# meyerls/FruitNeRF

Measured on AMD Instinct MI355X. Metric: train rays/sec, fruit_nerf on synthetic apple 800x800, higher is better.
Workload: dtype f32 fwd (MLP GEMMs: 3-piece bf16 split, 6 products, ~2^-24) / 2-piece bwd (dX, dW: 3 products, ~2^-17; its forward recompute 3-piece); everything else f32

## Files before the change

### fruitnerf_amd/csrc/field_bf16.hpp

```cpp
#pragma once
#include "field_layers.hpp"

namespace fnr {

using bf16x8 = __attribute__((ext_vector_type(8))) __bf16;
using f32x8 = __attribute__((ext_vector_type(8))) float;

enum { MLP_FP32 = 0, MLP_BF16 = 1, MLP_BF16X3 = 3 };

template <class Cfg>
struct BfImage {
  static constexpr int NL = Cfg::NLAYERS;
  static constexpr int nib_used(int l) { return l == Cfg::L_COL0 ? Cfg::HB : Cfg::nib(l); }
  static constexpr int nkb(int l) { return (nib_used(l) + 1) / 2; }
  static constexpr int nkbT(int l) { return (Cfg::nob(l) + 1) / 2; }
  static constexpr bool hasT(int l) { return l != Cfg::L_SEM0; }
  static constexpr int fblocks(int l) { return Cfg::nob(l) * nkb(l); }
  static constexpr int tblocks(int l) { return hasT(l) ? nib_used(l) * nkbT(l) : 0; }
  static constexpr int foff(int l) {
    int o = 0;
    for (int i = 0; i < l; ++i) o += fblocks(i);
    return o;
  }
  static constexpr int F_TOTAL = foff(NL);
  static constexpr int toff(int l) {
    int o = F_TOTAL;
    for (int i = 0; i < l; ++i) o += tblocks(i);
    return o;
  }
  static constexpr int BLOCKS = toff(NL);
  static constexpr size_t piece_elems() { return (size_t)BLOCKS * 64 * 8; }
  static constexpr size_t bytes(int ns) { return (size_t)ns * piece_elems() * 2; }
};
constexpr int BF_MAX_PIECES = 3;

__device__ __forceinline__ __bf16 bf_piece(float w, int p) {
  const __bf16 a = (__bf16)w;
  if (p == 0) return a;
  const float r1 = w - (float)a;
  const __bf16 b = (__bf16)r1;
  if (p == 1) return b;
  return (__bf16)(r1 - (float)b);
}

template <class Cfg>
__device__ __forceinline__ void pack_field_weights_bf16_block(const FieldPtrs& p, int ns, __bf16* __restrict__ image,
                                                              int block) {
  using Img = BfImage<Cfg>;
  const int idx = block * 256 + threadIdx.x;
  if (idx >= Img::BLOCKS * 64) return;
  const int blk = idx >> 6, lane = idx & 63;
  const int i = lane & 15, g = lane >> 4;
  float w[8];
  if (blk < Img::F_TOTAL) {
    int l = 0;
#pragma unroll
    for (int q = 1; q < Cfg::NLAYERS; ++q)
      if (blk >= Img::foff(q)) l = q;
    const int local = blk - Img::foff(l);
    const int nkb = Img::nkb(l), kb = local % nkb, ob = local / nkb;
    const int out = 16 * ob + i;
#pragma unroll
    for (int e = 0; e < 8; ++e) {
      const int ib = 2 * kb + (e >> 2);
      const int col = (ib < Img::nib_used(l)) ? kmap<Cfg>(Cfg::km(l), ib, g, e & 3, Cfg::in_dim(l)) : -1;
      w[e] = (out < Cfg::out_dim(l) && col >= 0) ? p.w[l][out * Cfg::in_dim(l) + col] : 0.0f;
    }
  } else {
    int l = 0;
#pragma unroll
    for (int q = 1; q < Cfg::NLAYERS; ++q)
      if (blk >= Img::toff(q)) l = q;
    const int local = blk - Img::toff(l);
    const int nk = Img::nkbT(l), kb = local % nk, ib = local / nk;
    const int col = kmap<Cfg>(Cfg::km(l), ib, i >> 2, i & 3, Cfg::in_dim(l));
#pragma unroll
    for (int e = 0; e < 8; ++e) {
      const int ob = 2 * kb + (e >> 2);
      const int out = 16 * ob + 4 * g + (e & 3);
      w[e] = (ob < Cfg::nob(l) && out < Cfg::out_dim(l) && col >= 0) ? p.w[l][out * Cfg::in_dim(l) + col] : 0.0f;
    }
  }
  for (int pc = 0; pc < ns; ++pc) {
    bf16x8 v;
#pragma unroll
    for (int e = 0; e < 8; ++e) v[e] = bf_piece(w[e], pc);
    reinterpret_cast<bf16x8*>(image)[(size_t)pc * Img::BLOCKS * 64 + idx] = v;
  }
}

template <class Cfg>
__global__ __launch_bounds__(256) void k_pack_field_weights_bf16(FieldPtrs p, int ns, __bf16* __restrict__ image) {
  pack_field_weights_bf16_block<Cfg>(p, ns, image, blockIdx.x);
}
template <class Cfg>
constexpr int pack_field_weights_bf16_blocks() { return (BfImage<Cfg>::BLOCKS * 64 + 255) / 256; }

template <class Cfg>
static inline void launch_pack_field_weights_bf16(const FieldPtrs& p, int ns, __bf16* image, hipStream_t st) {
  hipLaunchKernelGGL((k_pack_field_weights_bf16<Cfg>), dim3(pack_field_weights_bf16_blocks<Cfg>()), dim3(256), 0, st, p, ns,
                     image);
}

template <class Cfg>
__global__ __launch_bounds__(256) void k_prepare_field(FieldPtrs p, float* __restrict__ packed, int ns,
                                                       __bf16* __restrict__ image, RaysDev rays,
                                                       const float* __restrict__ embedding,
                                                       const float* __restrict__ mean_embedding,
                                                       float* __restrict__ ray_bias, int nb_pack, int nb_pack16) {
  int b = blockIdx.x;
  if (b < nb_pack) {
    pack_field_weights_block<Cfg>(p, packed, b);
    return;
  }
  b -= nb_pack;
  if (b < nb_pack16) {
    pack_field_weights_bf16_block<Cfg>(p, ns, image, b);
    return;
  }
  b -= nb_pack16;
  color_ray_bias_block<Cfg, true>(p, nullptr, rays, embedding, mean_embedding, ray_bias, b,
                                  (int)gridDim.x - nb_pack - nb_pack16);
}
template <class Cfg>
static inline void launch_prepare_field(const FieldPtrs& p, float* packed, int ns, __bf16* image, const RaysDev& rays,
                                        const float* embedding, const float* mean_embedding, float* ray_bias,
                                        hipStream_t st) {
  const int nb_pack = pack_field_weights_blocks<Cfg>();
  const int nb_pack16 = ns > 0 ? pack_field_weights_bf16_blocks<Cfg>() : 0;
  const long long nb_bias = color_ray_bias_blocks(rays);
  hipLaunchKernelGGL((k_prepare_field<Cfg>), dim3((unsigned)(nb_pack + nb_pack16 + nb_bias)), dim3(256), 0, st, p, packed, ns,
                     image, rays, embedding, mean_embedding, ray_bias, nb_pack, nb_pack16);
}

template <class Cfg, class Segs, int NS>
struct BfLds {
  using Img = BfImage<Cfg>;
  static constexpr int blocks(int s) { return Segs::isT(s) ? Img::tblocks(Segs::layer(s)) : Img::fblocks(Segs::layer(s)); }
  static constexpr int off(int s) {
    int o = 0;
    for (int i = 0; i < s; ++i) o += blocks(i) * NS;
    return o;
  }
  static constexpr int FRAGS = off(Segs::N);
  static constexpr int BYTES = FRAGS * 1024;
  static constexpr int find(int layer, bool isT) {
    for (int i = 0; i < Segs::N; ++i)
      if (Segs::layer(i) == layer && Segs::isT(i) == isT) return i;
    return -1;
  }
  template <int LAYER, bool IS_T>
  __device__ static __forceinline__ const bf16x8* seg(const bf16x8* lds) {
    constexpr int s = find(LAYER, IS_T);
    static_assert(s >= 0, "layer not staged by this kernel");
    return lds + off(s) * 64;
  }
  template <int LAYER, bool IS_T>
  static constexpr int seg_blocks() { return blocks(find(LAYER, IS_T)); }
  static constexpr int chunk_begin(int c) { return off(c / NS) * 64 + (c % NS) * blocks(c / NS) * 64; }
  static constexpr long long chunk_src(int c) {
    const int s = c / NS, pc = c % NS;
    return (long long)pc * Img::BLOCKS * 64 + (Segs::isT(s) ? Img::toff(Segs::layer(s)) : Img::foff(Segs::layer(s))) * 64;
  }
  template <int THREADS>
  __device__ static __forceinline__ void stage(bf16x8* __restrict__ lds, const __bf16* __restrict__ image) {
    constexpr int T = FRAGS * 64, NCH = Segs::N * NS;
    constexpr int PER = (T + THREADS - 1) / THREADS;
    static_assert(PER <= 32, "staging batch too large");
    const f32x4* img = reinterpret_cast<const f32x4*>(image);
    f32x4* dst = reinterpret_cast<f32x4*>(lds);
    f32x4 v[PER];
#pragma unroll
    for (int u = 0; u < PER; ++u) {
      const int f = (int)threadIdx.x + u * THREADS;
      long long delta = chunk_src(0) - chunk_begin(0);
#pragma unroll
      for (int c = 1; c < NCH; ++c) delta = (f >= chunk_begin(c)) ? chunk_src(c) - chunk_begin(c) : delta;
      if (f < T) v[u] = img[f + delta];
    }
#pragma unroll
    for (int u = 0; u < PER; ++u) {
      const int f = (int)threadIdx.x + u * THREADS;
      if (f < T) dst[f] = v[u];
    }
  }
};

template <class Cfg, int L, int NS, int THREADS>
__device__ __forceinline__ void bf_build_T(bf16x8* __restrict__ lds, const float* __restrict__ packed) {
  constexpr int NIB = Cfg::nib(L), NKT = (Cfg::nob(L) + 1) / 2, TB = NIB * NKT;
  for (int idx = threadIdx.x; idx < TB * 64; idx += THREADS) {
    const int blk = idx >> 6, lane = idx & 63;
    const int i = lane & 15, g = lane >> 4;
    const int kb = blk % NKT, ib = blk / NKT;
    float w[8];
#pragma unroll
    for (int e = 0; e < 8; ++e) {
      const int ob = 2 * kb + (e >> 2), row = 4 * g + (e & 3);
      w[e] = ob < Cfg::nob(L) ? packed[Cfg::woff(L) + ((ob * NIB + ib) * 64 + swz_slot(row, i >> 2)) * 4 + (i & 3)] : 0.0f;
    }
#pragma unroll
    for (int pc = 0; pc < NS; ++pc) {
      bf16x8 v;
#pragma unroll
      for (int e = 0; e < 8; ++e) v[e] = bf_piece(w[e], pc);
      lds[pc * TB * 64 + idx] = v;
    }
  }
}

using bf_f32x2 = __attribute__((ext_vector_type(2))) float;
using bf_bf16x2 = __attribute__((ext_vector_type(2))) __bf16;
__device__ __forceinline__ unsigned cvt_pk_bf16(float lo, float hi) {
  const bf_f32x2 v = {lo, hi};
  return __builtin_bit_cast(unsigned, __builtin_convertvector(v, bf_bf16x2));
}
using bf_u32x4 = __attribute__((ext_vector_type(4))) unsigned;
template <int NS>
__device__ __forceinline__ void bf_split(const f32x8 v, bf16x8 (&p)[NS]) {
  bf_u32x4 out[NS];
#pragma unroll
  for (int d = 0; d < 4; ++d) {
    float a = v[2 * d], b = v[2 * d + 1];
#pragma unroll
    for (int pc = 0; pc < NS; ++pc) {
      const unsigned w = cvt_pk_bf16(a, b);
      out[pc][d] = w;
      if (pc + 1 < NS) {
        a -= __builtin_bit_cast(float, w << 16);
        b -= __builtin_bit_cast(float, w & 0xffff0000u);
      }
    }
  }
#pragma unroll
  for (int pc = 0; pc < NS; ++pc) p[pc] = __builtin_bit_cast(bf16x8, out[pc]);
}
template <int NS>
__device__ __forceinline__ void bf_split_half(const f32x4 v, bf16x8 (&p)[NS]) {
  bf_u32x4 out[NS];
#pragma unroll
  for (int d = 0; d < 2; ++d) {
    float a = v[2 * d], b = v[2 * d + 1];
#pragma unroll
    for (int pc = 0; pc < NS; ++pc) {
      const unsigned w = cvt_pk_bf16(a, b);
      out[pc][d] = w;
      if (pc + 1 < NS) {
        a -= __builtin_bit_cast(float, w << 16);
        b -= __builtin_bit_cast(float, w & 0xffff0000u);
      }
    }
  }
#pragma unroll
  for (int pc = 0; pc < NS; ++pc) {
    out[pc][2] = out[pc][3] = 0u;
    p[pc] = __builtin_bit_cast(bf16x8, out[pc]);
  }
}

template <int NS, int NB>
__device__ __forceinline__ void bf_operand(const f32x4 (&act)[NB], bf16x8 (&x)[(NB + 1) / 2][NS]) {
#pragma unroll
  for (int kb = 0; kb < (NB + 1) / 2; ++kb) {
    if (2 * kb + 1 < NB) {
      f32x8 v;
#pragma unroll
      for (int e = 0; e < 4; ++e) {
        v[e] = act[2 * kb][e];
        v[4 + e] = act[(2 * kb + 1 < NB) ? 2 * kb + 1 : 0][e];
      }
      bf_split<NS>(v, x[kb]);
    } else {
      bf_split_half<NS>(act[2 * kb], x[kb]);
    }
  }
}

template <int NS, int NOB, int NKB>
__device__ __forceinline__ void bf_layer_acc(const bf16x8* __restrict__ seg, const bf16x8 (&xa)[NKB][NS],
                                             const bf16x8 (&xb)[NKB][NS], f32x4 (&oa)[NOB], f32x4 (&ob_)[NOB], int lane) {
  constexpr int PB = NOB * NKB * 64;
#pragma unroll
  for (int kb = 0; kb < NKB; ++kb) {
#pragma unroll
    for (int ob = 0; ob < NOB; ++ob) {
      bf16x8 w[NS];
#pragma unroll
      for (int pc = 0; pc < NS; ++pc) w[pc] = seg[pc * PB + (ob * NKB + kb) * 64 + lane];
#pragma unroll
      for (int s = NS - 1; s >= 0; --s)
#pragma unroll
        for (int pw = 0; pw <= s; ++pw) {
          oa[ob] = __builtin_amdgcn_mfma_f32_16x16x32_bf16(w[pw], xa[kb][s - pw], oa[ob], 0, 0, 0);
          ob_[ob] = __builtin_amdgcn_mfma_f32_16x16x32_bf16(w[pw], xb[kb][s - pw], ob_[ob], 0, 0, 0);
        }
    }
  }
}

template <int NS, int NOB, int NIB>
__device__ __forceinline__ void bf_layer(const bf16x8* __restrict__ seg, const float* __restrict__ B,
                                         const f32x4 (&ina)[NIB], const f32x4 (&inb)[NIB], f32x4 (&oa)[NOB],
                                         f32x4 (&ob_)[NOB], int lane) {
  const int g = lane >> 4;
#pragma unroll
  for (int ob = 0; ob < NOB; ++ob) oa[ob] = ob_[ob] = *reinterpret_cast<const f32x4*>(B + 16 * ob + 4 * g);
  bf16x8 xa[(NIB + 1) / 2][NS], xb[(NIB + 1) / 2][NS];
  bf_operand<NS, NIB>(ina, xa);
  bf_operand<NS, NIB>(inb, xb);
  bf_layer_acc<NS, NOB, (NIB + 1) / 2>(seg, xa, xb, oa, ob_, lane);
}

template <int NS, int NIBO, int NOB>
__device__ __forceinline__ void bf_layer_T(const bf16x8* __restrict__ segT, const f32x4 (&Ga)[NOB], const f32x4 (&Gb)[NOB],
                                           f32x4 (&oa)[NIBO], f32x4 (&ob_)[NIBO], int lane) {
#pragma unroll
  for (int ib = 0; ib < NIBO; ++ib) oa[ib] = ob_[ib] = f32x4{0.f, 0.f, 0.f, 0.f};
  bf16x8 xa[(NOB + 1) / 2][NS], xb[(NOB + 1) / 2][NS];
  bf_operand<NS, NOB>(Ga, xa);
  bf_operand<NS, NOB>(Gb, xb);
  bf_layer_acc<NS, NIBO, (NOB + 1) / 2>(segT, xa, xb, oa, ob_, lane);
}

template <int NS, int NOB, int NKB>
__device__ __forceinline__ void bf_layer_acc1(const bf16x8* __restrict__ seg, const bf16x8 (&x)[NKB][NS], f32x4 (&o)[NOB],
                                              int lane) {
  constexpr int PB = NOB * NKB * 64, T = NOB * NKB;
  bf16x8 w[2][NS];
  auto load = [&](int t, bf16x8 (&dst)[NS]) {
    const int kb = t / NOB, ob = t % NOB;
#pragma unroll
    for (int pc = 0; pc < NS; ++pc) dst[pc] = seg[pc * PB + (ob * NKB + kb) * 64 + lane];
  };
  load(0, w[0]);
#pragma unroll
  for (int t = 0; t < T; ++t) {
    if (t + 1 < T) load(t + 1, w[(t + 1) & 1]);
    const int kb = t / NOB, ob = t % NOB;
#pragma unroll
    for (int s = NS - 1; s >= 0; --s)
#pragma unroll
      for (int pw = 0; pw <= s; ++pw)
        o[ob] = __builtin_amdgcn_mfma_f32_16x16x32_bf16(w[t & 1][pw], x[kb][s - pw], o[ob], 0, 0, 0);
    __builtin_amdgcn_sched_barrier(0);
  }
}
template <int NS, int NOB, int NIB>
__device__ __forceinline__ void bf_layer1(const bf16x8* __restrict__ seg, const float* __restrict__ B,
                                          const f32x4 (&in)[NIB], f32x4 (&o)[NOB], int lane) {
  const int g = lane >> 4;
#pragma unroll
  for (int ob = 0; ob < NOB; ++ob) o[ob] = *reinterpret_cast<const f32x4*>(B + 16 * ob + 4 * g);
  bf16x8 x[(NIB + 1) / 2][NS];
  bf_operand<NS, NIB>(in, x);
  bf_layer_acc1<NS, NOB, (NIB + 1) / 2>(seg, x, o, lane);
}
template <int NS, int NIBO, int NOB>
__device__ __forceinline__ void bf_layer_T1(const bf16x8* __restrict__ segT, const f32x4 (&G)[NOB], f32x4 (&o)[NIBO],
                                            int lane) {
#pragma unroll
  for (int ib = 0; ib < NIBO; ++ib) o[ib] = f32x4{0.f, 0.f, 0.f, 0.f};
  bf16x8 x[(NOB + 1) / 2][NS];
  bf_operand<NS, NOB>(G, x);
  bf_layer_acc1<NS, NIBO, (NOB + 1) / 2>(segT, x, o, lane);
}

size_t field_bf16_image_bytes();
int field_mlp_fwd_bf16(int cfg, int mode, const FieldPtrs& p, const float* packed, void* image_ws, const float* ray_bias,
                       const RaysDev& rd, int S, long long N, const float2* feats, const uint8_t* selector, float* density,
                       float* rgb, float* logit, float* geo_out, float* h_buf, hipStream_t st);
int field_mlp_fwd_sem_big_bf16(int mode, const FieldPtrs& p, void* image_ws, const float* packed, long long N,
                               const float* h_buf, float* logit, hipStream_t st);
int field_mlp_bwd_sem_big_bf16(int mode, const FieldPtrs& p, void* image_ws, const float* packed, long long N,
                               const float* h_saved, const float* d_logit, float* partials, long long blocks,
                               hipStream_t st, float* d_h_semgrad = nullptr);
namespace pw {
struct BwdArgs {
  const float* packed;
  const __bf16* image;
  const float* ray_bias;
  RaysDev rd;
  int S;
  long long N;
  const float2* feats;
  const float* h_saved;
  const uint8_t* selector;
  const float *d_density, *d_rgb, *d_logit;
  float2* d_feats;
  float *d_h, *gsum_tile, *gsum_extra, *partials;
  long long blocks;
  hipStream_t st;
};
}
int field_mlp_bwd_pw(int cfg, int mode, int branch, const pw::BwdArgs& a, const float2* jac, float4* d_pos);

}
```

### fruitnerf_amd/csrc/field_mlp_bf16.hip

```cpp
#include <type_traits>

#include "field_bf16.hpp"

namespace fnr {

template <class Cfg>
struct SegsFwdAll {
  static constexpr int N = Cfg::NLAYERS;
  static constexpr int layer(int i) { return i; }
  static constexpr bool isT(int) { return false; }
};

template <class Cfg>
struct SegsFwdBaseColor {
  static constexpr int N = 5;
  static constexpr int layer(int i) {
    return i == 0 ? Cfg::L_BASE0 : i == 1 ? Cfg::L_BASE1 : i == 2 ? Cfg::L_COL0 : i == 3 ? Cfg::L_COL1 : Cfg::L_COL2;
  }
  static constexpr bool isT(int) { return false; }
};

__device__ __forceinline__ void load_hash_block(const float2* __restrict__ feats, long long N, long long nn, int g,
                                                f32x4 (&x0)[2]) {
#pragma unroll
  for (int m = 0; m < 4; ++m) {
    const float2 v = feats[(size_t)(4 * m + g) * N + nn];
    x0[m >> 1][2 * (m & 1)] = v.x;
    x0[m >> 1][2 * (m & 1) + 1] = v.y;
  }
}

template <int N>
__device__ __forceinline__ void relu2_(f32x4 (&a)[N], f32x4 (&b)[N]) {
  relu_(a);
  relu_(b);
}

template <class Cfg, int NS, int WAVES, bool WITH_SEM>
__global__ __launch_bounds__(64 * WAVES, WAVES / 4) void k_field_mlp_fwd_bf16(
    const float* __restrict__ packed, const __bf16* __restrict__ image, const float* __restrict__ ray_bias, RaysDev rays,
    int S, long long N, const float2* __restrict__ feats, const uint8_t* __restrict__ selector,
    float* __restrict__ density, float* __restrict__ rgb, float* __restrict__ logit, float* __restrict__ geo_out,
    float* __restrict__ h_buf) {
  constexpr int HB = Cfg::HB;
  static_assert(HB == 1 || HB == 2, "built shapes");
  static_assert(!WITH_SEM || (HB == 1 && Cfg::NSEM == 2), "all-in-one kernel: `fruit_nerf` shape");
  using Segs = typename std::conditional<WITH_SEM, SegsFwdAll<Cfg>, SegsFwdBaseColor<Cfg>>::type;
  using Lds = BfLds<Cfg, Segs, NS>;
  extern __shared__ __attribute__((aligned(16))) unsigned char smem[];
  bf16x8* lds = reinterpret_cast<bf16x8*>(smem);
  float* bias = reinterpret_cast<float*>(smem + Lds::BYTES);
  Lds::template stage<64 * WAVES>(lds, image);
  for (int i = threadIdx.x; i < Cfg::B_TOTAL; i += blockDim.x) bias[i] = packed[Cfg::W_TOTAL + i];
  __syncthreads();
  const int lane = threadIdx.x & 63, wave = threadIdx.x >> 6;
  const int j = lane & 15, g = lane >> 4;
  const long long n_pairs = (N + 31) / 32;
  for (long long pr = (long long)blockIdx.x * WAVES + wave; pr < n_pairs; pr += (long long)gridDim.x * WAVES) {
    asm volatile("" ::: "memory");
    const long long na = pr * 32 + j, nb = na + 16;
    const bool va = na < N, vb = nb < N;
    const long long nna = va ? na : N - 1, nnb = vb ? nb : N - 1;
    const long long raya = nna / S, rayb = nnb / S;

    f32x4 ha[HB], hb[HB];
    {
      f32x4 xa[2], xb[2], a1a[4], a1b[4];
      load_hash_block(feats, N, nna, g, xa);
      load_hash_block(feats, N, nnb, g, xb);
      bf_layer<NS, 4, 2>(Lds::template seg<Cfg::L_BASE0, false>(lds), bias + Cfg::boff(Cfg::L_BASE0), xa, xb, a1a, a1b, lane);
      relu2_(a1a, a1b);
      bf_layer<NS, HB, 4>(Lds::template seg<Cfg::L_BASE1, false>(lds), bias + Cfg::boff(Cfg::L_BASE1), a1a, a1b, ha, hb, lane);
    }
    if constexpr (WITH_SEM) {
      f32x4 s1a[4], s1b[4], s2a[4], s2b[4], hda[1], hdb[1];
      bf_layer<NS, 4, 1>(Lds::template seg<Cfg::L_SEM0, false>(lds), bias + Cfg::boff(Cfg::L_SEM0), ha, hb, s1a, s1b, lane);
      relu2_(s1a, s1b);
      bf_layer<NS, 4, 4>(Lds::template seg<Cfg::L_SEM1, false>(lds), bias + Cfg::boff(Cfg::L_SEM1), s1a, s1b, s2a, s2b, lane);
      bf_layer<NS, 1, 4>(Lds::template seg<Cfg::L_HEAD, false>(lds), bias + Cfg::boff(Cfg::L_HEAD), s2a, s2b, hda, hdb, lane);
      if (g == 0 && va) logit[na] = hda[0][0];
      if (g == 0 && vb) logit[nb] = hdb[0][0];
    }
    {
      f32x4 c1a[4], c1b[4], c2a[4], c2b[4], c3a[1], c3b[1];
#pragma unroll
      for (int ob = 0; ob < 4; ++ob) {
        c1a[ob] = *reinterpret_cast<const f32x4*>(ray_bias + (size_t)raya * 64 + 16 * ob + 4 * g);
        c1b[ob] = *reinterpret_cast<const f32x4*>(ray_bias + (size_t)rayb * 64 + 16 * ob + 4 * g);
      }
      {
        bf16x8 xa[1][NS], xb[1][NS];
        bf_operand<NS, HB>(ha, xa);
        bf_operand<NS, HB>(hb, xb);
        bf_layer_acc<NS, 4, 1>(Lds::template seg<Cfg::L_COL0, false>(lds), xa, xb, c1a, c1b, lane);
      }
      relu2_(c1a, c1b);
      bf_layer<NS, 4, 4>(Lds::template seg<Cfg::L_COL1, false>(lds), bias + Cfg::boff(Cfg::L_COL1), c1a, c1b, c2a, c2b, lane);
      relu2_(c2a, c2b);
      bf_layer<NS, 1, 4>(Lds::template seg<Cfg::L_COL2, false>(lds), bias + Cfg::boff(Cfg::L_COL2), c2a, c2b, c3a, c3b, lane);
      auto finish = [&](long long n, bool valid, const f32x4 (&h)[HB], const f32x4 (&c3)[1]) {
        if (!valid) return;
#pragma unroll
        for (int b = 0; b < HB; ++b) {
          if (h_buf) *reinterpret_cast<f32x4*>(h_buf + (size_t)n * (16 * HB) + 16 * b + 4 * g) = h[b];
          if (geo_out) {
#pragma unroll
            for (int r = 0; r < 4; ++r) {
              const int k = 16 * b + 4 * g + r;
              if (k >= 1 && k <= Cfg::GEO) geo_out[(size_t)n * Cfg::GEO + (k - 1)] = h[b][r];
            }
          }
        }
        if (g == 0) {
          const bool sel = selector ? (selector[n] != 0) : true;
          density[n] = sel ? expf(h[0][0]) : 0.0f;
          rgb[3 * n + 0] = 1.0f / (1.0f + expf(-c3[0][0]));
          rgb[3 * n + 1] = 1.0f / (1.0f + expf(-c3[0][1]));
          rgb[3 * n + 2] = 1.0f / (1.0f + expf(-c3[0][2]));
        }
      };
      finish(na, va, ha, c3a);
      finish(nb, vb, hb, c3b);
    }
  }
}

template <int N>
__device__ __forceinline__ void zero_vec_bf(f32x4 (&a)[N]) {
#pragma unroll
  for (int b = 0; b < N; ++b) a[b] = f32x4{0.f, 0.f, 0.f, 0.f};
}

template <class Cfg>
struct SegsBigP1 {
  static constexpr int N = 2;
  static constexpr int layer(int i) { return i == 0 ? Cfg::L_SEM0 : Cfg::L_SEM1; }
  static constexpr bool isT(int) { return false; }
};
template <class Cfg>
struct SegsBigP2 {
  static constexpr int N = 2;
  static constexpr int layer(int i) { return i == 0 ? Cfg::L_HEAD : Cfg::L_SEM2; }
  static constexpr bool isT(int) { return true; }
};
template <class Cfg>
struct SegsBigP4 {
  static constexpr int N = 1;
  static constexpr int layer(int) { return Cfg::L_SEM1; }
  static constexpr bool isT(int) { return true; }
};

constexpr int CS_LD = 72;
constexpr int CS_ROWS = 128;
template <int NS>
constexpr int cs_words() { return 2 * NS * CS_ROWS * CS_LD; }

template <int NS, int NB>
__device__ __forceinline__ void cs_write(uint32_t* __restrict__ arr, int row0, const f32x4 (&a)[NB], int lane, int wave) {
  const int j = lane & 15, g = lane >> 4;
  __bf16* base = reinterpret_cast<__bf16*>(arr);
#pragma unroll
  for (int blk = 0; blk < NB; ++blk)
#pragma unroll
    for (int r = 0; r < 4; ++r) {
      float v = a[blk][r];
#pragma unroll
      for (int pc = 0; pc < NS; ++pc) {
        const __bf16 pv = (__bf16)v;
        base[(size_t)((pc * CS_ROWS + row0 + 16 * blk + 4 * g + r) * (2 * CS_LD)) + 16 * wave + j] = pv;
        if (pc + 1 < NS) v -= (float)pv;
      }
    }
}

template <int NS, int NOBW>
__device__ __forceinline__ void cs_dw(const uint32_t* __restrict__ sG, const uint32_t* __restrict__ sX, int ob0,
                                      int ob_step, int ib, f32x4 (&acc)[NOBW], int lane) {
  const int i = lane & 15, g = lane >> 4;
  constexpr int T = 4 * NOBW;
  bf16x8 ga[2][NS], xb[NS];
  auto load_g = [&](int t, bf16x8 (&dst)[NS]) {
    const int kk = t / NOBW, ob = ob0 + (t % NOBW) * ob_step;
#pragma unroll
    for (int pc = 0; pc < NS; ++pc)
      dst[pc] = *reinterpret_cast<const bf16x8*>(sG + (pc * CS_ROWS + 16 * ob + i) * CS_LD + 16 * kk + 4 * g);
  };
  load_g(0, ga[0]);
#pragma unroll
  for (int t = 0; t < T; ++t) {
    const int kk = t / NOBW, s = t % NOBW;
    if (s == 0) {
#pragma unroll
      for (int pc = 0; pc < NS; ++pc)
        xb[pc] = *reinterpret_cast<const bf16x8*>(sX + (pc * CS_ROWS + 16 * ib + i) * CS_LD + 16 * kk + 4 * g);
    }
    if (t + 1 < T) load_g(t + 1, ga[(t + 1) & 1]);
#pragma unroll
    for (int sp = NS - 1; sp >= 0; --sp)
#pragma unroll
      for (int pg = 0; pg <= sp; ++pg)
        acc[s] = __builtin_amdgcn_mfma_f32_16x16x32_bf16(ga[t & 1][pg], xb[sp - pg], acc[s], 0, 0, 0);
    __builtin_amdgcn_sched_barrier(0);
  }
}
template <int NS>
__device__ __forceinline__ void cs_bias(const uint32_t* __restrict__ sG, int ob, f32x4& bacc, int lane) {
  const int i = lane & 15, g = lane >> 4;
  bf16x8 ones;
#pragma unroll
  for (int e = 0; e < 8; ++e) ones[e] = (__bf16)1.0f;
#pragma unroll
  for (int kk = 0; kk < 4; ++kk)
#pragma unroll
    for (int pc = NS - 1; pc >= 0; --pc) {
      const bf16x8 ga = *reinterpret_cast<const bf16x8*>(sG + (pc * CS_ROWS + 16 * ob + i) * CS_LD + 16 * kk + 4 * g);
      bacc = __builtin_amdgcn_mfma_f32_16x16x32_bf16(ga, ones, bacc, 0, 0, 0);
    }
}
__device__ __forceinline__ void store_dw_block(float* __restrict__ W, int ob, int ib, int nib_stride, const f32x4& acc,
                                               int lane) {
  const int jn = lane & 15, g = lane >> 4;
#pragma unroll
  for (int r = 0; r < 4; ++r)
    W[((ob * nib_stride + ib) * 64 + swz_slot(4 * g + r, jn >> 2)) * 4 + (jn & 3)] = acc[r];
}
__device__ __forceinline__ void store_bias_block(float* __restrict__ B, int ob, const f32x4& bacc, int lane) {
  if ((lane & 15) == 0) {
    const int g = lane >> 4;
#pragma unroll
    for (int r = 0; r < 4; ++r) B[16 * ob + 4 * g + r] = bacc[r];
  }
}

template <class Cfg, int NSF, int NS, bool SEMGRAD = false, class... DH>
__global__ __launch_bounds__(512, 2) void k_field_mlp_bwd_sem_big_bf16(
    const float* __restrict__ packed, const __bf16* __restrict__ image, const float* __restrict__ w_sem2,
    const float* __restrict__ b_sem2, long long N, const float* __restrict__ h_saved, const float* __restrict__ d_logit,
    float* __restrict__ partials, DH... d_h_semgrad) {
  static_assert(sizeof...(DH) == (SEMGRAD ? 1 : 0), "d_h comes with SEMGRAD");
  static_assert(Cfg::NSEM == 3 && Cfg::HB == 2 && Cfg::SEMB == 8, "fruit_nerf_big semantic shape");
  constexpr int WAVES = 8, THREADS = 64 * WAVES;
  constexpr int LS0 = Cfg::L_SEM0, LS1 = Cfg::L_SEM1, LS2 = Cfg::L_SEM2, LH = Cfg::L_HEAD;
  static_assert(LS1 == LS0 + 1 && LS2 == LS1 + 1 && LH == LS2 + 1, "the branch's layers are adjacent in the fp32 image");
  using P1 = BfLds<Cfg, SegsBigP1<Cfg>, NSF>;
  using P2 = BfLds<Cfg, SegsBigP2<Cfg>, NS>;
  using P4 = BfLds<Cfg, SegsBigP4<Cfg>, NS>;
  constexpr int REGION = cs_words<NS>() * 4;
  static_assert(P1::BYTES <= REGION && P2::BYTES <= REGION && P4::BYTES <= REGION, "phase weights exceed the shared region");
  extern __shared__ __attribute__((aligned(16))) unsigned char smem[];
  bf16x8* wl = reinterpret_cast<bf16x8*>(smem);
  uint32_t* sG = reinterpret_cast<uint32_t*>(smem);
  uint32_t* sX = sG + NS * CS_ROWS * CS_LD;
  float* fbias = reinterpret_cast<float*>(smem + REGION);
  float* vhead = fbias + 256;
  for (int i = threadIdx.x; i < 256; i += THREADS) fbias[i] = packed[Cfg::W_TOTAL + Cfg::boff(LS0) + i];
  const int lane0 = threadIdx.x & 63, wave = threadIdx.x >> 6;

  f32x4 acc0[2], acc1[8], acc2[4], accV[1];
  f32x4 b0 = {0.f, 0.f, 0.f, 0.f}, b1 = b0, b2 = b0;
  zero_vec_bf(acc0);
  zero_vec_bf(acc1);
  zero_vec_bf(acc2);
  zero_vec_bf(accV);

  const long long n_batches = (N + 127) / 128;
  for (long long batch = blockIdx.x; batch < n_batches; batch += gridDim.x) {
    asm volatile("" ::: "memory");
    int lane = lane0;
    asm volatile("" : "+v"(lane));
    const int j = lane & 15, g = lane >> 4;
    const long long n = batch * 128 + 16 * wave + j;
    const bool valid = n < N;
    const long long nn = valid ? n : N - 1;
    f32x4 h[2];
    h[0] = *reinterpret_cast<const f32x4*>(h_saved + (size_t)nn * 32 + 4 * g);
    h[1] = *reinterpret_cast<const f32x4*>(h_saved + (size_t)nn * 32 + 16 + 4 * g);
    f32x4 Gl[1];
    Gl[0] = f32x4{0.f, 0.f, 0.f, 0.f};
    if (g == 0 && valid) Gl[0][0] = d_logit[n];

    __syncthreads();
    P1::template stage<THREADS>(wl, image);
    __syncthreads();
    f32x4 s1[8], s2[8];
    bf_layer1<NSF, 8, 2>(P1::template seg<LS0, false>(wl), fbias, h, s1, lane);
    relu_(s1);
    bf_layer1<NSF, 8, 8>(P1::template seg<LS1, false>(wl), fbias + 128, s1, s2, lane);
    relu_(s2);
    __syncthreads();
    bf16x8* wl2 = reinterpret_cast<bf16x8*>(sX);
    static_assert(P2::BYTES <= NS * CS_ROWS * CS_LD * 4, "phase-2 fragments must fit the X half");
    P2::template stage<THREADS>(wl2, image);
    __syncthreads();
    f32x4 Gs2[8];
    {
      f32x4 Gs3[4];
      bf_layer_T1<NS, 4, 1>(P2::template seg<LH, true>(wl2), Gl, Gs3, lane);
      cs_write<NS, 4>(sG, 0, Gs3, lane, wave);
      cs_write<NS, 1>(sG, 64, Gl, lane, wave);
      bf_layer_T1<NS, 8, 4>(P2::template seg<LS2, true>(wl2), Gs3, Gs2, lane);
    }
#pragma unroll
    for (int b = 0; b < 8; ++b)
#pragma unroll
      for (int r = 0; r < 4; ++r) Gs2[b][r] = (s2[b][r] > 0.0f) ? Gs2[b][r] : 0.0f;
    __syncthreads();
    cs_write<NS, 8>(sX, 0, s2, lane, wave);
    __syncthreads();
    cs_dw<NS, 4>(sG, sX, 0, 1, wave, acc2, lane);
    cs_dw<NS, 1>(sG, sX, 4, 0, wave, accV, lane);
    if (wave < 4) cs_bias<NS>(sG, wave, b2, lane);
    if (wave == 4) cs_bias<NS>(sG, 4, b2, lane);
    __syncthreads();
    cs_write<NS, 8>(sG, 0, Gs2, lane, wave);
    cs_write<NS, 8>(sX, 0, s1, lane, wave);
    __syncthreads();
    cs_dw<NS, 8>(sG, sX, 0, 1, wave, acc1, lane);
    cs_bias<NS>(sG, wave, b1, lane);
    __syncthreads();
    P4::template stage<THREADS>(wl, image);
    __syncthreads();
    f32x4 Gs1[8];
    bf_layer_T1<NS, 8, 8>(P4::template seg<LS1, true>(wl), Gs2, Gs1, lane);
#pragma unroll
    for (int b = 0; b < 8; ++b)
#pragma unroll
      for (int r = 0; r < 4; ++r) Gs1[b][r] = (s1[b][r] > 0.0f) ? Gs1[b][r] : 0.0f;
    __syncthreads();
    cs_write<NS, 8>(sG, 0, Gs1, lane, wave);
    {
      f32x4 hx[2];
      hx[0] = *reinterpret_cast<const f32x4*>(h_saved + (size_t)nn * 32 + 4 * g);
      hx[1] = *reinterpret_cast<const f32x4*>(h_saved + (size_t)nn * 32 + 16 + 4 * g);
      cs_write<NS, 2>(sX, 0, hx, lane, wave);
    }
    __syncthreads();
    cs_dw<NS, 2>(sG, sX, wave >> 1, 4, wave & 1, acc0, lane);
    cs_bias<NS>(sG, wave, b0, lane);
    if constexpr (SEMGRAD) {
      constexpr int T0_BYTES = NS * Cfg::nib(LS0) * ((Cfg::nob(LS0) + 1) / 2) * 1024;
      static_assert(T0_BYTES <= REGION, "sem0's transposed fragments exceed the shared region");
      __syncthreads();
      bf_build_T<Cfg, LS0, NS, THREADS>(wl, packed);
      __syncthreads();
      f32x4 Gh[2];
      bf_layer_T1<NS, 2, 8>(wl, Gs1, Gh, lane);
      if (g == 0) Gh[0][0] = 0.0f;
      if (valid) {
        float* const d_h = only(d_h_semgrad...);
#pragma unroll
        for (int b = 0; b < 2; ++b) {
          f32x4* row = reinterpret_cast<f32x4*>(d_h + (size_t)n * 32 + 16 * b + 4 * g);
          *row = *row + Gh[b];
        }
      }
    }
  }

  const int lane = lane0;
  float* part = partials + (size_t)blockIdx.x * (Cfg::W_TOTAL + Cfg::B_TOTAL);
  float* pb = part + Cfg::W_TOTAL;
#pragma unroll
  for (int s = 0; s < 2; ++s) store_dw_block(part + Cfg::woff(LS0), (wave >> 1) + 4 * s, wave & 1, 2, acc0[s], lane);
#pragma unroll
  for (int s = 0; s < 8; ++s) store_dw_block(part + Cfg::woff(LS1), s, wave, 8, acc1[s], lane);
#pragma unroll
  for (int s = 0; s < 4; ++s) store_dw_block(part + Cfg::woff(LS2), s, wave, 8, acc2[s], lane);
  store_bias_block(pb + Cfg::boff(LS0), wave, b0, lane);
  store_bias_block(pb + Cfg::boff(LS1), wave, b1, lane);
  if (wave < 4) store_bias_block(pb + Cfg::boff(LS2), wave, b2, lane);
  __syncthreads();
  if ((lane >> 4) == 0) vhead[16 * wave + (lane & 15)] = accV[0][0];
  if (wave == 4 && lane == 0) vhead[128] = b2[0];
  for (int i = threadIdx.x; i < Cfg::nob(LH) * Cfg::nib(LH) * 256; i += THREADS) part[Cfg::woff(LH) + i] = 0.0f;
  for (int i = threadIdx.x; i < 16; i += THREADS) pb[Cfg::boff(LH) + i] = 0.0f;
  __syncthreads();
  if (threadIdx.x < 64) {
    const int k = threadIdx.x;
    float dw = b_sem2[k] * vhead[128];
    for (int m = 0; m < 128; ++m) dw = fmaf(w_sem2[k * 128 + m], vhead[m], dw);
    const int ib = k >> 4, kk = k & 15;
    part[Cfg::woff(LH) + (ib * 64 + swz_slot(0, kk >> 2)) * 4 + (kk & 3)] = dw;
    if (k == 0) pb[Cfg::boff(LH)] = vhead[128];
  }
}

template <class Cfg>
struct SegsBigF2 {
  static constexpr int N = 2;
  static constexpr int layer(int i) { return i == 0 ? Cfg::L_SEM2 : Cfg::L_HEAD; }
  static constexpr bool isT(int) { return false; }
};

template <class Cfg, int NS, int WAVES>
__global__ __launch_bounds__(64 * WAVES, WAVES / 4) void k_field_mlp_fwd_sem_big_bf16(
    const float* __restrict__ packed, const __bf16* __restrict__ image, long long N, const float* __restrict__ h_buf,
    float* __restrict__ logit) {
  static_assert(Cfg::NSEM == 3 && Cfg::HB == 2 && Cfg::SEMB == 8, "fruit_nerf_big semantic shape");
  constexpr int THREADS = 64 * WAVES;
  constexpr int LS0 = Cfg::L_SEM0, LS1 = Cfg::L_SEM1, LS2 = Cfg::L_SEM2, LH = Cfg::L_HEAD;
  using F1 = BfLds<Cfg, SegsBigP1<Cfg>, NS>;
  using F2 = BfLds<Cfg, SegsBigF2<Cfg>, NS>;
  constexpr int REGION = F1::BYTES > F2::BYTES ? F1::BYTES : F2::BYTES;
  extern __shared__ __attribute__((aligned(16))) unsigned char smem[];
  bf16x8* wl = reinterpret_cast<bf16x8*>(smem);
  float* fbias = reinterpret_cast<float*>(smem + REGION);
  for (int i = threadIdx.x; i < 336; i += THREADS) fbias[i] = packed[Cfg::W_TOTAL + Cfg::boff(LS0) + i];
  const int lane = threadIdx.x & 63, wave = threadIdx.x >> 6;
  const int j = lane & 15, g = lane >> 4;
  const long long per_batch = 16 * WAVES;
  const long long n_batches = (N + per_batch - 1) / per_batch;
  for (long long batch = blockIdx.x; batch < n_batches; batch += gridDim.x) {
    asm volatile("" ::: "memory");
    const long long n = batch * per_batch + 16 * wave + j;
    const bool valid = n < N;
    const long long nn = valid ? n : N - 1;
    f32x4 h[2];
    h[0] = *reinterpret_cast<const f32x4*>(h_buf + (size_t)nn * 32 + 4 * g);
    h[1] = *reinterpret_cast<const f32x4*>(h_buf + (size_t)nn * 32 + 16 + 4 * g);
    __syncthreads();
    F1::template stage<THREADS>(wl, image);
    __syncthreads();
    f32x4 s1[8], s2[8];
    bf_layer1<NS, 8, 2>(F1::template seg<LS0, false>(wl), fbias, h, s1, lane);
    relu_(s1);
    bf_layer1<NS, 8, 8>(F1::template seg<LS1, false>(wl), fbias + 128, s1, s2, lane);
    relu_(s2);
    __syncthreads();
    F2::template stage<THREADS>(wl, image);
    __syncthreads();
    f32x4 s3[4], hd[1];
    bf_layer1<NS, 4, 8>(F2::template seg<LS2, false>(wl), fbias + 256, s2, s3, lane);
    bf_layer1<NS, 1, 4>(F2::template seg<LH, false>(wl), fbias + 320, s3, hd, lane);
    if (g == 0 && valid) logit[n] = hd[0][0];
  }
}

int field_mlp_fwd_sem_big_bf16(int mode, const FieldPtrs& p, void* image_ws, const float* packed, long long N,
                               const float* h_buf, float* logit, hipStream_t st) {
  using Cfg = FieldCfgBig;
  __bf16* image = reinterpret_cast<__bf16*>(image_ws);
  constexpr int WAVES = 8;
  const long long n_batches = (N + 16 * WAVES - 1) / (16 * WAVES);
  long long blocks = n_batches;
  if (blocks > (long long)device_cu_count()) blocks = device_cu_count();
  auto launch = [&](int once, auto kern, int bytes) -> int {
    if (once) return once;
    hipLaunchKernelGGL(kern, dim3((unsigned)blocks), dim3(64 * WAVES), bytes, st, packed, image, N, h_buf, logit);
    FNR_LAUNCH_CHECK();
    return FNR_OK;
  };
  if (mode == MLP_BF16) {
    constexpr int bytes = BfLds<Cfg, SegsBigP1<Cfg>, 1>::BYTES + 336 * 4;
    constexpr auto kern = k_field_mlp_fwd_sem_big_bf16<Cfg, 1, WAVES>;
    return launch(ensure_dyn_lds<kern>(bytes), kern, bytes);
  }
  constexpr int bytes = BfLds<Cfg, SegsBigP1<Cfg>, 3>::BYTES + 336 * 4;
  static_assert(bytes <= 160 * 1024, "fruit_nerf_big forward fragments exceed the LDS");
  constexpr auto kern = k_field_mlp_fwd_sem_big_bf16<Cfg, 3, WAVES>;
  return launch(ensure_dyn_lds<kern>(bytes), kern, bytes);
}

int field_mlp_bwd_sem_big_bf16(int mode, const FieldPtrs& p, void* image_ws, const float* packed, long long N,
                               const float* h_saved, const float* d_logit, float* partials, long long blocks,
                               hipStream_t st, float* d_h_semgrad) {
  using Cfg = FieldCfgBig;
  __bf16* image = reinterpret_cast<__bf16*>(image_ws);
  auto launch = [&](int once, auto kern, int bytes) -> int {
    if (once) return once;
    hipLaunchKernelGGL(kern, dim3((unsigned)blocks), dim3(512), bytes, st, packed, image, p.w[Cfg::L_SEM2], p.b[Cfg::L_SEM2],
                       N, h_saved, d_logit, partials);
    FNR_LAUNCH_CHECK();
    return FNR_OK;
  };
  if (d_h_semgrad) {
    auto launch_sg = [&](int once, auto kern, int bytes) -> int {
      if (once) return once;
      hipLaunchKernelGGL(kern, dim3((unsigned)blocks), dim3(512), bytes, st, packed, image, p.w[Cfg::L_SEM2],
                         p.b[Cfg::L_SEM2], N, h_saved, d_logit, partials, d_h_semgrad);
      FNR_LAUNCH_CHECK();
      return FNR_OK;
    };
    if (mode == MLP_BF16) {
      constexpr int bytes = cs_words<1>() * 4 + (256 + 144) * 4;
      constexpr auto kern = k_field_mlp_bwd_sem_big_bf16<Cfg, 1, 1, true, float*>;
      return launch_sg(ensure_dyn_lds<kern>(bytes), kern, bytes);
    }
    constexpr int bytes = cs_words<2>() * 4 + (256 + 144) * 4;
    constexpr auto kern = k_field_mlp_bwd_sem_big_bf16<Cfg, 3, 2, true, float*>;
    return launch_sg(ensure_dyn_lds<kern>(bytes), kern, bytes);
  }
  if (mode == MLP_BF16) {
    constexpr int bytes = cs_words<1>() * 4 + (256 + 144) * 4;
    constexpr auto kern = k_field_mlp_bwd_sem_big_bf16<Cfg, 1, 1>;
    return launch(ensure_dyn_lds<kern>(bytes), kern, bytes);
  }
  constexpr int bytes = cs_words<2>() * 4 + (256 + 144) * 4;
  static_assert(bytes <= 160 * 1024, "fruit_nerf_big semantic branch exceeds the LDS");
  constexpr auto kern = k_field_mlp_bwd_sem_big_bf16<Cfg, 3, 2>;
  return launch(ensure_dyn_lds<kern>(bytes), kern, bytes);
}

template <class Cfg, int NS>
static int fwd_launch_bf16(const float* packed, const __bf16* image, const float* ray_bias, const RaysDev& rd, int S,
                           long long N, const float2* feats, const uint8_t* selector, float* density, float* rgb,
                           float* logit, float* geo_out, float* h_buf, hipStream_t st) {
  constexpr bool WITH_SEM = Cfg::NSEM == 2;
  using Segs = typename std::conditional<WITH_SEM, SegsFwdAll<Cfg>, SegsFwdBaseColor<Cfg>>::type;
  using Lds = BfLds<Cfg, Segs, NS>;
  constexpr int WAVES = 8;
  constexpr int bytes = Lds::BYTES + Cfg::B_TOTAL * 4;
  static_assert(bytes <= 160 * 1024, "forward fragments exceed the LDS");
  constexpr auto kern = k_field_mlp_fwd_bf16<Cfg, NS, WAVES, WITH_SEM>;
  const int once = ensure_dyn_lds<kern>(bytes);
  if (once) return once;
  const long long n_pairs = (N + 31) / 32;
  long long blocks = (n_pairs + WAVES - 1) / WAVES;
  const long long max_blocks = (long long)device_cu_count() * (bytes <= 80 * 1024 ? 2 : 1);
  if (blocks > max_blocks) blocks = max_blocks;
  hipLaunchKernelGGL(kern, dim3((unsigned)blocks), dim3(64 * WAVES), bytes, st, packed, image, ray_bias, rd, S, N, feats,
                     selector, density, rgb, logit, geo_out, h_buf);
  FNR_LAUNCH_CHECK();
  return FNR_OK;
}

int field_mlp_fwd_bf16(int cfg, int mode, const FieldPtrs& p, const float* packed, void* image_ws, const float* ray_bias,
                       const RaysDev& rd, int S, long long N, const float2* feats, const uint8_t* selector, float* density,
                       float* rgb, float* logit, float* geo_out, float* h_buf, hipStream_t st) {
  __bf16* image = reinterpret_cast<__bf16*>(image_ws);
#define FNR_FWD16(C, NSV) \
  fwd_launch_bf16<C, NSV>(packed, image, ray_bias, rd, S, N, feats, selector, density, rgb, logit, geo_out, h_buf, st)
  if (cfg == 0) return mode == MLP_BF16 ? FNR_FWD16(FieldCfgBase, 1) : FNR_FWD16(FieldCfgBase, 3);
  return mode == MLP_BF16 ? FNR_FWD16(FieldCfgBig, 1) : FNR_FWD16(FieldCfgBig, 3);
#undef FNR_FWD16
}

size_t field_bf16_image_bytes() {
  const size_t a = BfImage<FieldCfgBase>::bytes(BF_MAX_PIECES), b = BfImage<FieldCfgBig>::bytes(BF_MAX_PIECES);
  return (a > b ? a : b) + 256;
}

}
```

Before: 6.468 million.

## Fuse ReLU and bf16 split into forward MLP layer epilogue, raise waves

The forward field MLP now splits each layer's f32 output into bf16 pieces (with optional ReLU) as soon as each pair of output blocks is done, and feeds those directly into the next layer. This replaces the separate relu pass and the bf_operand conversion. The hidden state h is split once and reused by both the semantic and color branches instead of being re-split. The store of h and density is moved earlier so the f32 h registers can be released. The all-in-one 3-piece kernel also goes from 8 to 12 waves per block, which trades register pressure for occupancy.

```diff
diff --git a/fruitnerf_amd/csrc/field_bf16.hpp b/fruitnerf_amd/csrc/field_bf16.hpp
--- a/fruitnerf_amd/csrc/field_bf16.hpp
+++ b/fruitnerf_amd/csrc/field_bf16.hpp
@@ -309,6 +309,73 @@
   bf_operand<NS, NIB>(ina, xa);
   bf_operand<NS, NIB>(inb, xb);
   bf_layer_acc<NS, NOB, (NIB + 1) / 2>(seg, xa, xb, oa, ob_, lane);
+}
+
+template <int NS, bool RELU, bool ONE>
+__device__ __forceinline__ void bf_fwd_split(const f32x4& b0, const f32x4& b1, bf16x8 (&p)[NS]) {
+  bf_u32x4 out[NS];
+#pragma unroll
+  for (int d = 0; d < (ONE ? 2 : 4); ++d) {
+    float a = d < 2 ? b0[2 * d] : b1[2 * d - 4], b = d < 2 ? b0[2 * d + 1] : b1[2 * d - 3];
+    if (RELU) {
+      a = fmaxf(a, 0.0f);
+      b = fmaxf(b, 0.0f);
+    }
+#pragma unroll
+    for (int pc = 0; pc < NS; ++pc) {
+      const unsigned w = cvt_pk_bf16(a, b);
+      out[pc][d] = w;
+      if (pc + 1 < NS) {
+        a -= __builtin_bit_cast(float, w << 16);
+        b -= __builtin_bit_cast(float, w & 0xffff0000u);
+        asm("" : "+v"(a), "+v"(b));
+      }
+    }
+  }
+#pragma unroll
+  for (int pc = 0; pc < NS; ++pc) {
+    if (ONE) out[pc][2] = out[pc][3] = 0u;
+    p[pc] = __builtin_bit_cast(bf16x8, out[pc]);
+  }
+}
+
+template <int NOB>
+__device__ __forceinline__ void bf_fwd_bias(const float* __restrict__ B, f32x4 (&oa)[NOB], f32x4 (&ob_)[NOB], int lane) {
+  const int g = lane >> 4;
+#pragma unroll
+  for (int ob = 0; ob < NOB; ++ob) oa[ob] = ob_[ob] = *reinterpret_cast<const f32x4*>(B + 16 * ob + 4 * g);
+}
+
+template <int NS, int NOB, int NKB, bool RELU, bool SPLIT>
+__device__ __forceinline__ void bf_fwd_layer(const bf16x8* __restrict__ seg, const bf16x8 (&xa)[NKB][NS],
+                                             const bf16x8 (&xb)[NKB][NS], f32x4 (&oa)[NOB], f32x4 (&ob_)[NOB],
+                                             bf16x8 (&ya)[(NOB + 1) / 2][NS], bf16x8 (&yb)[(NOB + 1) / 2][NS], int lane) {
+  constexpr int PB = NOB * NKB * 64;
+#pragma unroll
+  for (int kb = 0; kb < NKB; ++kb) {
+#pragma unroll
+    for (int ob = 0; ob < NOB; ++ob) {
+      bf16x8 w[NS];
+#pragma unroll
+      for (int pc = 0; pc < NS; ++pc) w[pc] = seg[pc * PB + (ob * NKB + kb) * 64 + lane];
+#pragma unroll
+      for (int s = NS - 1; s >= 0; --s)
+#pragma unroll
+        for (int pw = 0; pw <= s; ++pw) {
+          oa[ob] = __builtin_amdgcn_mfma_f32_16x16x32_bf16(w[pw], xa[kb][s - pw], oa[ob], 0, 0, 0);
+          ob_[ob] = __builtin_amdgcn_mfma_f32_16x16x32_bf16(w[pw], xb[kb][s - pw], ob_[ob], 0, 0, 0);
+        }
+      if (SPLIT && kb == NKB - 1 && ((ob & 1) || ob == NOB - 1)) {
+        if (ob & 1) {
+          bf_fwd_split<NS, RELU, false>(oa[ob - 1], oa[ob], ya[ob >> 1]);
+          bf_fwd_split<NS, RELU, false>(ob_[ob - 1], ob_[ob], yb[ob >> 1]);
+        } else {
+          bf_fwd_split<NS, RELU, true>(oa[ob], oa[ob], ya[ob >> 1]);
+          bf_fwd_split<NS, RELU, true>(ob_[ob], ob_[ob], yb[ob >> 1]);
+        }
+      }
+    }
+  }
 }
 
 template <int NS, int NIBO, int NOB>
diff --git a/fruitnerf_amd/csrc/field_mlp_bf16.hip b/fruitnerf_amd/csrc/field_mlp_bf16.hip
--- a/fruitnerf_amd/csrc/field_mlp_bf16.hip
+++ b/fruitnerf_amd/csrc/field_mlp_bf16.hip
@@ -28,12 +28,6 @@
     x0[m >> 1][2 * (m & 1)] = v.x;
     x0[m >> 1][2 * (m & 1) + 1] = v.y;
   }
-}
-
-template <int N>
-__device__ __forceinline__ void relu2_(f32x4 (&a)[N], f32x4 (&b)[N]) {
-  relu_(a);
-  relu_(b);
 }
 
 template <class Cfg, int NS, int WAVES, bool WITH_SEM>
@@ -63,64 +57,76 @@
     const long long nna = va ? na : N - 1, nnb = vb ? nb : N - 1;
     const long long raya = nna / S, rayb = nnb / S;
 
-    f32x4 ha[HB], hb[HB];
+    auto finish_h = [&](long long n, bool valid, const f32x4 (&h)[HB]) {
+      if (!valid) return;
+#pragma unroll
+      for (int b = 0; b < HB; ++b) {
+        if (h_buf) *reinterpret_cast<f32x4*>(h_buf + (size_t)n * (16 * HB) + 16 * b + 4 * g) = h[b];
+        if (geo_out) {
+#pragma unroll
+          for (int r = 0; r < 4; ++r) {
+            const int k = 16 * b + 4 * g + r;
+            if (k >= 1 && k <= Cfg::GEO) geo_out[(size_t)n * Cfg::GEO + (k - 1)] = h[b][r];
+          }
+        }
+      }
+      if (g == 0) {
+        const bool sel = selector ? (selector[n] != 0) : true;
+        density[n] = sel ? expf(h[0][0]) : 0.0f;
+      }
+    };
+    bf16x8 hxa[1][NS], hxb[1][NS];
     {
-      f32x4 xa[2], xb[2], a1a[4], a1b[4];
+      f32x4 xa[2], xb[2], a1a[4], a1b[4], ha[HB], hb[HB];
+      bf16x8 x0a[1][NS], x0b[1][NS], y1a[2][NS], y1b[2][NS];
       load_hash_block(feats, N, nna, g, xa);
       load_hash_block(feats, N, nnb, g, xb);
-      bf_layer<NS, 4, 2>(Lds::template seg<Cfg::L_BASE0, false>(lds), bias + Cfg::boff(Cfg::L_BASE0), xa, xb, a1a, a1b, lane);
-      relu2_(a1a, a1b);
-      bf_layer<NS, HB, 4>(Lds::template seg<Cfg::L_BASE1, false>(lds), bias + Cfg::boff(Cfg::L_BASE1), a1a, a1b, ha, hb, lane);
-    }
+      bf_fwd_split<NS, false, false>(xa[0], xa[1], x0a[0]);
+      bf_fwd_split<NS, false, false>(xb[0], xb[1], x0b[0]);
+      bf_fwd_bias<4>(bias + Cfg::boff(Cfg::L_BASE0), a1a, a1b, lane);
+      bf_fwd_layer<NS, 4, 1, true, true>(Lds::template seg<Cfg::L_BASE0, false>(lds), x0a, x0b, a1a, a1b, y1a, y1b, lane);
+      bf_fwd_bias<HB>(bias + Cfg::boff(Cfg::L_BASE1), ha, hb, lane);
+      bf_fwd_layer<NS, HB, 2, false, true>(Lds::template seg<Cfg::L_BASE1, false>(lds), y1a, y1b, ha, hb, hxa, hxb, lane);
+      finish_h(na, va, ha);
+      finish_h(nb, vb, hb);
+    }
+    bf16x8 none[1][NS];
     if constexpr (WITH_SEM) {
       f32x4 s1a[4], s1b[4], s2a[4], s2b[4], hda[1], hdb[1];
-      bf_layer<NS, 4, 1>(Lds::template seg<Cfg::L_SEM0, false>(lds), bias + Cfg::boff(Cfg::L_SEM0), ha, hb, s1a, s1b, lane);
-      relu2_(s1a, s1b);
-      bf_layer<NS, 4, 4>(Lds::template seg<Cfg::L_SEM1, false>(lds), bias + Cfg::boff(Cfg::L_SEM1), s1a, s1b, s2a, s2b, lane);
-      bf_layer<NS, 1, 4>(Lds::template seg<Cfg::L_HEAD, false>(lds), bias + Cfg::boff(Cfg::L_HEAD), s2a, s2b, hda, hdb, lane);
+      bf16x8 y1a[2][NS], y1b[2][NS], y2a[2][NS], y2b[2][NS];
+      bf_fwd_bias<4>(bias + Cfg::boff(Cfg::L_SEM0), s1a, s1b, lane);
+      bf_fwd_layer<NS, 4, 1, true, true>(Lds::template seg<Cfg::L_SEM0, false>(lds), hxa, hxb, s1a, s1b, y1a, y1b, lane);
+      bf_fwd_bias<4>(bias + Cfg::boff(Cfg::L_SEM1), s2a, s2b, lane);
+      bf_fwd_layer<NS, 4, 2, false, true>(Lds::template seg<Cfg::L_SEM1, false>(lds), y1a, y1b, s2a, s2b, y2a, y2b, lane);
+      bf_fwd_bias<1>(bias + Cfg::boff(Cfg::L_HEAD), hda, hdb, lane);
+      bf_fwd_layer<NS, 1, 2, false, false>(Lds::template seg<Cfg::L_HEAD, false>(lds), y2a, y2b, hda, hdb, none, none, lane);
       if (g == 0 && va) logit[na] = hda[0][0];
       if (g == 0 && vb) logit[nb] = hdb[0][0];
     }
     {
       f32x4 c1a[4], c1b[4], c2a[4], c2b[4], c3a[1], c3b[1];
+      bf16x8 y1a[2][NS], y1b[2][NS], y2a[2][NS], y2b[2][NS];
 #pragma unroll
       for (int ob = 0; ob < 4; ++ob) {
         c1a[ob] = *reinterpret_cast<const f32x4*>(ray_bias + (size_t)raya * 64 + 16 * ob + 4 * g);
         c1b[ob] = *reinterpret_cast<const f32x4*>(ray_bias + (size_t)rayb * 64 + 16 * ob + 4 * g);
       }
-      {
-        bf16x8 xa[1][NS], xb[1][NS];
-        bf_operand<NS, HB>(ha, xa);
-        bf_operand<NS, HB>(hb, xb);
-        bf_layer_acc<NS, 4, 1>(Lds::template seg<Cfg::L_COL0, false>(lds), xa, xb, c1a, c1b, lane);
-      }
-      relu2_(c1a, c1b);
-      bf_layer<NS, 4, 4>(Lds::template seg<Cfg::L_COL1, false>(lds), bias + Cfg::boff(Cfg::L_COL1), c1a, c1b, c2a, c2b, lane);
-      relu2_(c2a, c2b);
-      bf_layer<NS, 1, 4>(Lds::template seg<Cfg::L_COL2, false>(lds), bias + Cfg::boff(Cfg::L_COL2), c2a, c2b, c3a, c3b, lane);
-      auto finish = [&](long long n, bool valid, const f32x4 (&h)[HB], const f32x4 (&c3)[1]) {
-        if (!valid) return;
-#pragma unroll
-        for (int b = 0; b < HB; ++b) {
-          if (h_buf) *reinterpret_cast<f32x4*>(h_buf + (size_t)n * (16 * HB) + 16 * b + 4 * g) = h[b];
-          if (geo_out) {
-#pragma unroll
-            for (int r = 0; r < 4; ++r) {
-              const int k = 16 * b + 4 * g + r;
-              if (k >= 1 && k <= Cfg::GEO) geo_out[(size_t)n * Cfg::GEO + (k - 1)] = h[b][r];
-            }
-          }
-        }
-        if (g == 0) {
-          const bool sel = selector ? (selector[n] != 0) : true;
-          density[n] = sel ? expf(h[0][0]) : 0.0f;
-          rgb[3 * n + 0] = 1.0f / (1.0f + expf(-c3[0][0]));
-          rgb[3 * n + 1] = 1.0f / (1.0f + expf(-c3[0][1]));
-          rgb[3 * n + 2] = 1.0f / (1.0f + expf(-c3[0][2]));
+      bf_fwd_layer<NS, 4, 1, true, true>(Lds::template seg<Cfg::L_COL0, false>(lds), hxa, hxb, c1a, c1b, y1a, y1b, lane);
+      bf_fwd_bias<4>(bias + Cfg::boff(Cfg::L_COL1), c2a, c2b, lane);
+      bf_fwd_layer<NS, 4, 2, true, true>(Lds::template seg<Cfg::L_COL1, false>(lds), y1a, y1b, c2a, c2b, y2a, y2b, lane);
+      bf_fwd_bias<1>(bias + Cfg::boff(Cfg::L_COL2), c3a, c3b, lane);
+      bf_fwd_layer<NS, 1, 2, false, false>(Lds::template seg<Cfg::L_COL2, false>(lds), y2a, y2b, c3a, c3b, none, none, lane);
+      auto finish = [&](long long n, bool valid, const f32x4 (&c3)[1]) {
+        if (!valid || g != 0) return;
+#pragma unroll
+        for (int c = 0; c < 3; ++c) {
+          float d = 1.0f + expf(-c3[0][c]);
+          asm("" : "+v"(d));
+          rgb[3 * n + c] = 1.0f / d;
         }
       };
-      finish(na, va, ha, c3a);
-      finish(nb, vb, hb, c3b);
+      finish(na, va, c3a);
+      finish(nb, vb, c3b);
     }
   }
 }
@@ -508,7 +514,7 @@
   constexpr bool WITH_SEM = Cfg::NSEM == 2;
   using Segs = typename std::conditional<WITH_SEM, SegsFwdAll<Cfg>, SegsFwdBaseColor<Cfg>>::type;
   using Lds = BfLds<Cfg, Segs, NS>;
-  constexpr int WAVES = 8;
+  constexpr int WAVES = (WITH_SEM && NS == 3) ? 12 : 8;
   constexpr int bytes = Lds::BYTES + Cfg::B_TOTAL * 4;
   static_assert(bytes <= 160 * 1024, "forward fragments exceed the LDS");
   constexpr auto kern = k_field_mlp_fwd_bf16<Cfg, NS, WAVES, WITH_SEM>;
```

Result: no change. 6.518 million (median of 6 runs) (+0.8%).
